# dusk-network/plonk

Measured on AMD Instinct MI355X. Metric: prove() wall-clock (ms) at 2^20 gates, lower is better.
Workload: dtype u32 limbs (Fr 256-bit / Fp 384-bit Montgomery)

## Files before the change

### plonk_amd/csrc/msm.hip

```cpp
#include <cstdlib>

#include "plonk_internal.hpp"
#include "curve28.cuh"
#include "fr29.cuh"

namespace plonk {


static constexpr uint32_t MSM_KSL = 32;
static constexpr uint32_t MSM_CHUNK = 16;

__device__ __forceinline__ Fr ld_fr_g(const Fr* p) {
  const uint4* q = reinterpret_cast<const uint4*>(p);
  uint4 a = q[0], b = q[1];
  Fr r;
  r.l[0] = a.x; r.l[1] = a.y; r.l[2] = a.z; r.l[3] = a.w;
  r.l[4] = b.x; r.l[5] = b.y; r.l[6] = b.z; r.l[7] = b.w;
  return r;
}
__device__ __forceinline__ Fp ld_fp(const Fp* p) {
  const uint4* q = reinterpret_cast<const uint4*>(p);
  uint4 a = q[0], b = q[1], c = q[2];
  Fp r;
  r.l[0] = a.x; r.l[1] = a.y; r.l[2] = a.z; r.l[3] = a.w;
// ... 410 lines not shown
  G1RSlot* __restrict__ buckets = buckets_all + (uint64_t)kb * MSM_NB;
  __shared__ G1R sh[BS_G > 1 ? 128 : 32];
  if (blockIdx.x < fused) {
    __shared__ uint32_t found[3];
    const HeavyItem* __restrict__ list = heavy_list_all + (uint64_t)kb * MSM_NB;
    G1RSlot* __restrict__ seg_sum = seg_sum_all + (uint64_t)kb * seg_cap;
    const uint32_t t = threadIdx.x, q = t & 3, L = t >> 2;
    const uint32_t nitems = nheavy_all[2 * kb], nsegs = nheavy_all[2 * kb + 1];
    for (uint32_t sg = blockIdx.x; sg < nsegs; sg += fused) {
      for (uint32_t i = t; i < nitems; i += 128) {
        const HeavyItem it = list[i];
        if (sg >= it.seg_base && sg < it.seg_base + it.nseg) { found[0] = it.bucket; found[1] = sg - it.seg_base; found[2] = it.nseg; }
      }
      __syncthreads();
      const uint32_t b = found[0], j = found[1], nseg = found[2];
      const uint32_t beg = slice_off[b] + j * HEAVY_SEG, bend = slice_off[b + 1];
      G1R acc = G1R::identity();
      for (uint32_t r = 0; r < HEAVY_SEG / 32; ++r) {
        const uint32_t k = beg + L + 32 * r;
        if (k < bend) acc = g1r_add_quad(acc, ld_g1r(partial + k), q);
      }
      for (uint32_t d = 16; d >= 1; d >>= 1) {
        if (q == 0) sh[L] = acc;
        __syncthreads();
        if (L < d) acc = g1r_add_quad(acc, sh[L + d], q);
        __syncthreads();
      }
      if (t == 0) st_g1r(nseg == 1 ? buckets + b : seg_sum + sg, acc);
      __syncthreads();
    }
    return;
  }
  if (multi_list_all || dense_quad) {
    const uint32_t nmulti = dense_quad ? MSM_NB : nheavy_all[2 * MSM_MAX_BATCH + kb];
    const uint32_t* __restrict__ list = multi_list_all ? multi_list_all + (uint64_t)kb * MSM_NB : nullptr;
    const uint32_t q = threadIdx.x & 3;
    for (uint32_t i = ((blockIdx.x - fused) * blockDim.x + threadIdx.x) >> 2; i < nmulti; i += ((gridDim.x - fused) * blockDim.x) >> 2) {
      const uint32_t mb = dense_quad ? i : list[i];
      const uint32_t beg = slice_off[mb], end = slice_off[mb + 1];
      if (dense_quad) {
        if (end - beg > heavy_thresh || (direct && end - beg == 1)) continue;
        if (end == beg) { if (q == 0) st_g1r(buckets + mb, G1R::identity()); continue; }
      }
      G1R acc = ld_g1r(partial + beg);
      for (uint32_t k = beg + 1; k < end; ++k) acc = g1r_add_quad(acc, ld_g1r(partial + k), q);
      if (q == 0) st_g1r(buckets + mb, acc);
    }
    return;
  }
  const uint32_t t = (blockIdx.x - fused) * blockDim.x + threadIdx.x;
  const uint32_t b = t / BS_G, g = t % BS_G;
  G1R acc = G1R::identity();
  bool heavy = false;
  if (b < MSM_NB) {
    const uint32_t beg = slice_off[b], end = slice_off[b + 1];
    heavy = end - beg > heavy_thresh;
    if (direct && end - beg == 1) heavy = true;
    if (!heavy)
      for (uint32_t k = beg + g; k < end; k += BS_G) acc = acc.add(ld_g1r(partial + k));
  }
  for (int d = BS_G / 2; d >= 1; d >>= 1) {
    sh[threadIdx.x] = acc;
    __syncthreads();
    if ((int)g < d) acc = acc.add(sh[threadIdx.x + d]);
    __syncthreads();
  }
  if (g == 0 && b < MSM_NB && !heavy) st_g1r(buckets + b, acc);
}

// ... 785 lines not shown
  }
  prof_end(c, 2);
  HIP_TRY(hipGetLastError());
  return PLONK_OK;
#endif
#undef FINE_BEGIN
#undef FINE_END
}


}

#if PLONK_MSM_NB_BITS == 15
static uint64_t msm_slice_cap(const Ctx* c, uint64_t cap) {
  if (c->cfg.ksl >= 4) return (uint64_t)MSM_W * cap / c->cfg.ksl + MSM_NB_MAX + 1;
  const uint64_t nb15 = 1ull << 15;
  const uint64_t small = (uint64_t)MSM_W * cap / 4 < (uint64_t)MSM_W * nb15 ? (uint64_t)MSM_W * cap / 4 : (uint64_t)MSM_W * nb15;
  const uint64_t large = (uint64_t)MSM_W * cap / MSM_KSL;
  return (small > large ? small : large) + MSM_NB_MAX + 1;
}

int msm_sort_reserve_fixed(Ctx* c) {
  MsmWork& w = c->msm;
  constexpr int KB = MSM_MAX_BATCH;
  constexpr uint32_t COARSE = 2048;
  HIP_TRY(hipMalloc((void**)&w.coarse_cnt, sizeof(uint32_t) * COARSE * KB));
  HIP_TRY(hipMalloc((void**)&w.coarse_off, sizeof(uint32_t) * (COARSE + 1) * KB));
  HIP_TRY(hipMalloc((void**)&w.coarse_cur, sizeof(uint32_t) * COARSE * KB));
  HIP_TRY(hipMalloc((void**)&w.big_off, sizeof(uint32_t) * (COARSE + 1) * KB));
  HIP_TRY(hipMalloc((void**)&w.big_cnt, sizeof(uint32_t) * 2 * MSM_NB_MAX * KB));
  HIP_TRY(hipMalloc((void**)&w.full_off, sizeof(uint32_t) * (MSM_NB_MAX + 1) * KB));
  HIP_TRY(hipMalloc((void**)&w.part_list, sizeof(uint32_t) * (MSM_NB_MAX + 1) * KB));
  HIP_TRY(hipMalloc((void**)&w.multi_list, sizeof(uint32_t) * MSM_NB_MAX * KB));
  HIP_TRY(hipMalloc((void**)&w.layout, sizeof(uint32_t) * (2 * (MSM_NB_MAX / 1024) + (MSM_NB_MAX / 1024 + 1) * 132) * KB));
  return PLONK_OK;
}

int msm_reserve(Ctx* c, uint64_t m) {
  MsmWork& w = c->msm;
  constexpr int KB = MSM_MAX_BATCH;
  if (!w.fixed_ok) {
    for (void** q : {(void**)&w.offsets, (void**)&w.slice_off, (void**)&w.nheavy, &w.heavy_list, (void**)&w.coarse_cnt, (void**)&w.coarse_off,
                     (void**)&w.coarse_cur, (void**)&w.big_off, (void**)&w.big_cnt, (void**)&w.full_off, (void**)&w.part_list, (void**)&w.layout, (void**)&w.multi_list, &w.buckets, &w.chunk,
                     (void**)&w.result}) {
      if (*q) { (void)hipFree(*q); *q = nullptr; }
    }
    if (w.result_host) { (void)hipHostFree(w.result_host); w.result_host = nullptr; }
    HIP_TRY(hipMalloc((void**)&w.offsets, sizeof(uint32_t) * (MSM_NB_MAX + 1) * KB));
    HIP_TRY(hipMalloc((void**)&w.slice_off, sizeof(uint32_t) * (MSM_NB_MAX + 1) * KB));
    HIP_TRY(hipMalloc((void**)&w.nheavy, sizeof(uint32_t) * 4 * KB));
    HIP_TRY(hipMalloc((void**)&w.heavy_list, sizeof(HeavyItem) * MSM_NB_MAX * KB));
    { const int rc_s = msm_sort_reserve_fixed(c); if (rc_s) return rc_s; }
    HIP_TRY(hipMalloc((void**)&w.buckets, sizeof(G1RSlot) * MSM_NB_MAX * KB));
    HIP_TRY(hipMalloc((void**)&w.chunk, sizeof(G1RSlot) * (2 * (MSM_NB_MAX / 128) + 1024) * KB));
    HIP_TRY(hipMalloc((void**)&w.result, sizeof(G1) * MSM_BIT_SUMS * KB));
    HIP_TRY(hipHostMalloc((void**)&w.result_host, sizeof(G1) * MSM_BIT_SUMS * KB, hipHostMallocDefault));
    w.fixed_ok = true;
  }
  if (m > w.cap_m || msm_slice_cap(c, w.cap_m) > w.cap_slices) {
    const uint64_t cap = m > w.cap_m ? m : w.cap_m;
    HIP_TRY(hipStreamSynchronize(c->stream));
    w.cap_m = 0;
    for (void** q : {(void**)&w.tmp_words, (void**)&w.entries, (void**)&w.partial, &w.seg_sum}) {
      if (*q) { HIP_TRY(hipFree(*q)); *q = nullptr; }
    }
    HIP_TRY(hipMalloc((void**)&w.tmp_words, sizeof(uint64_t) * MSM_W * cap * KB));
    HIP_TRY(hipMalloc((void**)&w.entries, sizeof(uint32_t) * MSM_W * cap * KB));
// ... 115 lines not shown
```

### plonk_amd/csrc/msm_sort.hip

```cpp
#include "plonk_internal.hpp"
#include "fr29.cuh"

namespace plonk {
namespace PLONK_MSM_NS {

static constexpr uint32_t FINE_BITS = MSM_NB_BITS - 11;
static constexpr uint32_t COARSE = MSM_NB >> FINE_BITS;
#ifndef PLONK_SORT_TILE
#define PLONK_SORT_TILE 2048
#endif
static constexpr uint32_t TILE = PLONK_SORT_TILE;
static constexpr uint32_t SORT_T = 1024;
static constexpr uint32_t PER_T = TILE / SORT_T;
#ifndef PLONK_HIST_PER
#define PLONK_HIST_PER 2
#endif
static constexpr uint32_t HIST_PER = PLONK_HIST_PER;
static constexpr uint32_t HIST_TILE = SORT_T * HIST_PER;
static_assert(COARSE == 2 * SORT_T, "scan / reservation loops assume two coarse bins per thread");
static constexpr uint32_t IDX_BITS = 31 - FINE_BITS;
static constexpr uint32_t IDX_MASK = (1u << IDX_BITS) - 1;
static_assert(IDX_BITS + 1 + FINE_BITS == 32, "narrow intermediate word layout");
template <class WordT> struct SortWord;
template <> struct SortWord<uint32_t> {
// ... 94 lines not shown
__device__ __forceinline__ uint32_t block_exclusive_scan(uint32_t v, uint32_t* sh , uint32_t* total) {
  const uint32_t t = threadIdx.x;
  sh[t] = v;
  __syncthreads();
  for (uint32_t d = 1; d < SORT_T; d <<= 1) {
    const uint32_t x = t >= d ? sh[t - d] : 0;
    __syncthreads();
    sh[t] += x;
    __syncthreads();
  }
  const uint32_t incl = sh[t];
  *total = sh[SORT_T - 1];
  __syncthreads();
  return incl - v;
}

__device__ __forceinline__ void fine_exclusive_scan(const uint32_t* cnt, uint32_t* ex, uint32_t* sc, uint32_t* total) {
  constexpr uint32_t NF = 1u << FINE_BITS;
  const uint32_t t = threadIdx.x;
  const uint32_t v = t < NF ? cnt[t] : 0u;
  if (t < NF) sc[t] = v;
  __syncthreads();
  for (uint32_t d = 1; d < NF; d <<= 1) {
    const uint32_t x = (t < NF && t >= d) ? sc[t - d] : 0u;
    __syncthreads();
    if (t < NF) sc[t] += x;
    __syncthreads();
  }
  if (t < NF) ex[t] = sc[t] - v;
  *total = sc[NF - 1];
  __syncthreads();
}

static constexpr uint32_t BIG_LIMIT = 1u << 16;
static constexpr uint32_t BIG_CHUNK = 1u << 14;
__device__ __forceinline__ uint32_t big_chunks(uint32_t cnt) { return cnt > BIG_LIMIT ? (cnt + BIG_CHUNK - 1) / BIG_CHUNK : 0u; }

__global__ void __launch_bounds__(SORT_T) msm_coarse_scan_kernel(const uint32_t* __restrict__ coarse_cnt_all,
                                                                 uint32_t* __restrict__ coarse_off_all,
                                                                 uint32_t* __restrict__ coarse_cur_all,
                                                                 uint32_t* __restrict__ big_off_all, int kb0) {
  __shared__ uint32_t sh[SORT_T];
  const uint32_t* __restrict__ cnt = coarse_cnt_all + (uint64_t)(blockIdx.x + (uint32_t)kb0) * COARSE;
  uint32_t* __restrict__ off = coarse_off_all + (uint64_t)(blockIdx.x + (uint32_t)kb0) * (COARSE + 1);
  uint32_t* __restrict__ cur = coarse_cur_all + (uint64_t)(blockIdx.x + (uint32_t)kb0) * COARSE;
  uint32_t* __restrict__ big = big_off_all + (uint64_t)(blockIdx.x + (uint32_t)kb0) * (COARSE + 1);
  const uint32_t t = threadIdx.x;
  const uint32_t c0 = cnt[2 * t], c1 = cnt[2 * t + 1];
  uint32_t total;
  const uint32_t ex = block_exclusive_scan(c0 + c1, sh, &total);
  off[2 * t] = ex;
  off[2 * t + 1] = ex + c0;
  cur[2 * t] = 0;
  cur[2 * t + 1] = 0;
  if (t == SORT_T - 1) off[COARSE] = total;
  const uint32_t b0 = big_chunks(c0), b1 = big_chunks(c1);
  uint32_t btotal;
  const uint32_t bex = block_exclusive_scan(b0 + b1, sh, &btotal);
  big[2 * t] = bex;
  big[2 * t + 1] = bex + b0;
  if (t == SORT_T - 1) big[COARSE] = btotal;
}

static constexpr size_t PARTITION_LDS = ((size_t)TILE * MSM_W + 3 * COARSE) * sizeof(uint32_t);

template <int MODE, class WordT>
// ... 157 lines not shown
    }
  }
  __syncthreads();
  const TmpPlanes<WordT> tmp(tmp_all, kb, (uint64_t)MSM_W * bt.cap_m);
#pragma unroll
  for (uint32_t k = 0; k < P2_PER; ++k)
#pragma unroll
    for (uint32_t w = 0; w < P2_W; ++w)
      if (where[k][w] != 0xffffffffu) stage[loff[where[k][w] >> 16] + (where[k][w] & 0xffffu)] = word[k][w];
  __syncthreads();
  const uint32_t sub = t & 7;
  for (uint32_t bin = t >> 3; bin < COARSE; bin += P2_T / 8) {
    const uint32_t cnt = hist[bin], lo = loff[bin], gb = gbase[bin];
    for (uint32_t j = sub; j < cnt; j += 8) {
      const uint32_t lw = stage[lo + j];
      tmp.st(gb + j, SortWord<WordT>::make(lw >> 20, (lw >> 19) & 1u, (uint64_t)((lw >> 11) & 0xffu) * srs_n + base + (lw & 0x7ffu)));
    }
  }
}
#endif

#ifndef PLONK_FINE_T
#define PLONK_FINE_T 512
#endif
#ifndef PLONK_FINE_CACHE
#define PLONK_FINE_CACHE 20
#endif
static constexpr uint32_t FINE_T = PLONK_FINE_T;
static constexpr uint32_t FINE_CACHE = PLONK_FINE_CACHE;
template <class WordT>
__global__ void __launch_bounds__(FINE_T) msm_fine_kernel(MsmBatch bt, const uint32_t* __restrict__ coarse_off_all,
                                                          void* __restrict__ tmp_all,
                                                          uint32_t* __restrict__ entries_all,
                                                          uint32_t* __restrict__ offsets_all) {
  __shared__ uint32_t cnt[1u << FINE_BITS], start[1u << FINE_BITS], cur[1u << FINE_BITS], scan_tmp[1u << FINE_BITS];
  const int kb = (int)blockIdx.y + bt.kb0;
  const uint32_t bin = blockIdx.x, t = threadIdx.x;
  const uint32_t* __restrict__ coff = coarse_off_all + (uint64_t)kb * (COARSE + 1);
  const TmpPlanes<WordT> tmp(tmp_all, kb, (uint64_t)MSM_W * bt.cap_m);
  uint32_t* __restrict__ entries = entries_all + (uint64_t)kb * MSM_W * bt.cap_m;
  uint32_t* __restrict__ offsets = offsets_all + (uint64_t)kb * (MSM_NB + 1);
  const uint32_t beg = coff[bin], end = coff[bin + 1];
  if (end - beg > BIG_LIMIT) return;
  if (t < (1u << FINE_BITS)) { cnt[t] = 0; cur[t] = 0; }
  __syncthreads();
  WordT cache[FINE_CACHE > 0 ? FINE_CACHE : 1];
#pragma unroll
  for (uint32_t r = 0; r < FINE_CACHE; ++r) {
    const uint32_t j = beg + t + r * FINE_T;
    cache[r] = j < end ? tmp.ld(j) : (WordT)0;
  }
#pragma unroll
  for (uint32_t r = 0; r < FINE_CACHE; ++r)
    if (beg + t + r * FINE_T < end) atomicAdd(&cnt[SortWord<WordT>::fine(cache[r])], 1u);
  for (uint32_t j = beg + t + FINE_CACHE * FINE_T; j < end; j += FINE_T) atomicAdd(&cnt[tmp.ld_fine(j)], 1u);
  __syncthreads();
  {
    uint32_t total;
    fine_exclusive_scan(cnt, start, scan_tmp, &total);
    if (t < (1u << FINE_BITS)) {
      start[t] += beg;
      offsets[(bin << FINE_BITS) + t] = start[t];
    }
    if (t == 0 && bin == COARSE - 1) offsets[MSM_NB] = beg + total;
    __syncthreads();
  }
  __shared__ uint32_t sorted[(MSM_NB_BITS > 15 && FINE_CACHE > 0) ? FINE_T * FINE_CACHE : 1];
  const bool staged = MSM_NB_BITS > 15 && FINE_CACHE > 0 && end - beg <= FINE_T * FINE_CACHE;
  auto place = [&](WordT e) {
    const uint32_t f = SortWord<WordT>::fine(e);
    const uint32_t pos = start[f] + atomicAdd(&cur[f], 1u);
    if (staged) sorted[pos - beg] = SortWord<WordT>::entry(e);
    else entries[pos] = SortWord<WordT>::entry(e);
  };
#pragma unroll
  for (uint32_t r = 0; r < FINE_CACHE; ++r)
    if (beg + t + r * FINE_T < end) place(cache[r]);
  for (uint32_t j = beg + t + FINE_CACHE * FINE_T; j < end; j += FINE_T) place(tmp.ld(j));
  if (staged) {
    __syncthreads();
    for (uint32_t j = t; j < end - beg; j += FINE_T) entries[beg + j] = sorted[j];
  }
}

__device__ __forceinline__ bool big_item(const uint32_t* __restrict__ big, const uint32_t* __restrict__ coff, uint32_t w,
                                         uint32_t* bin, uint32_t* beg, uint32_t* end) {
  if (w >= big[COARSE]) return false;
  uint32_t lo = 0, hi = COARSE - 1;
  while (lo < hi) {
    const uint32_t mid = (lo + hi + 1) >> 1;
    if (big[mid] <= w) lo = mid; else hi = mid - 1;
  }
// ... 1 lines not shown
  const uint32_t b0 = coff[lo] + (w - big[lo]) * BIG_CHUNK, b1 = coff[lo + 1];
  *beg = b0;
  *end = b0 + BIG_CHUNK < b1 ? b0 + BIG_CHUNK : b1;
  return true;
}
static constexpr uint32_t BIG_T = 512;
static constexpr uint32_t BIG_PER = BIG_CHUNK / BIG_T;
template <class WordT>
__global__ void __launch_bounds__(BIG_T) msm_big_hist_kernel(MsmBatch bt, const uint32_t* __restrict__ coarse_off_all,
                                                             const uint32_t* __restrict__ big_off_all,
                                                             void* __restrict__ tmp_all, uint32_t* __restrict__ big_cnt_all) {
  __shared__ uint32_t cnt[1u << FINE_BITS];
  const int kb = (int)blockIdx.y + bt.kb0;
  const uint32_t* __restrict__ coff = coarse_off_all + (uint64_t)kb * (COARSE + 1);
  const uint32_t* __restrict__ big = big_off_all + (uint64_t)kb * (COARSE + 1);
  const TmpPlanes<WordT> tmp(tmp_all, kb, (uint64_t)MSM_W * bt.cap_m);
  const uint32_t t = threadIdx.x;
  for (uint32_t item = blockIdx.x;; item += gridDim.x) {
    uint32_t bin, beg, end;
    if (!big_item(big, coff, item, &bin, &beg, &end)) return;
    if (t < (1u << FINE_BITS)) cnt[t] = 0;
    __syncthreads();
    for (uint32_t j = beg + t; j < end; j += BIG_T) atomicAdd(&cnt[tmp.ld_fine(j)], 1u);
    __syncthreads();
    if (t < (1u << FINE_BITS) && cnt[t]) atomicAdd(&big_cnt_all[(uint64_t)kb * MSM_NB + (bin << FINE_BITS) + t], cnt[t]);
    __syncthreads();
  }
}
template <class WordT>
__global__ void __launch_bounds__(BIG_T) msm_big_scatter_kernel(MsmBatch bt, const uint32_t* __restrict__ coarse_off_all,
                                                                const uint32_t* __restrict__ big_off_all,
                                                                void* __restrict__ tmp_all,
                                                                const uint32_t* __restrict__ big_cnt_all, uint32_t* __restrict__ big_cur_all,
                                                                uint32_t* __restrict__ entries_all, uint32_t* __restrict__ offsets_all) {
  __shared__ uint32_t cnt[1u << FINE_BITS], base[1u << FINE_BITS], cur[1u << FINE_BITS], bin_cnt[1u << FINE_BITS], scan_tmp[1u << FINE_BITS];
  const int kb = (int)blockIdx.y + bt.kb0;
  const uint32_t* __restrict__ coff = coarse_off_all + (uint64_t)kb * (COARSE + 1);
  const uint32_t* __restrict__ big = big_off_all + (uint64_t)kb * (COARSE + 1);
  const TmpPlanes<WordT> tmp(tmp_all, kb, (uint64_t)MSM_W * bt.cap_m);
  uint32_t* __restrict__ entries = entries_all + (uint64_t)kb * MSM_W * bt.cap_m;
  uint32_t* __restrict__ offsets = offsets_all + (uint64_t)kb * (MSM_NB + 1);
  const uint32_t t = threadIdx.x;
  for (uint32_t item = blockIdx.x;; item += gridDim.x) {
    uint32_t bin, beg, end;
    if (!big_item(big, coff, item, &bin, &beg, &end)) return;
    const uint32_t* __restrict__ bcnt = big_cnt_all + (uint64_t)kb * MSM_NB + (bin << FINE_BITS);
    uint32_t* __restrict__ bcur = big_cur_all + (uint64_t)kb * MSM_NB + (bin << FINE_BITS);
    if (t < (1u << FINE_BITS)) { cnt[t] = 0; cur[t] = 0; }
    __syncthreads();
    WordT cache[BIG_PER];
#pragma unroll
    for (uint32_t r = 0; r < BIG_PER; ++r) {
      const uint32_t j = beg + t + r * BIG_T;
      cache[r] = j < end ? tmp.ld(j) : (WordT)0;
      if (j < end) atomicAdd(&cnt[SortWord<WordT>::fine(cache[r])], 1u);
    }
    __syncthreads();
    {
      const bool first = beg == coff[bin];
      if (t < (1u << FINE_BITS)) bin_cnt[t] = bcnt[t];
      __syncthreads();
      uint32_t total;
      fine_exclusive_scan(bin_cnt, base, scan_tmp, &total);
      if (t < (1u << FINE_BITS)) {
        const uint32_t run = coff[bin] + base[t];
        if (first) offsets[(bin << FINE_BITS) + t] = run;
        base[t] = run + (cnt[t] ? atomicAdd(&bcur[t], cnt[t]) : 0u);
      }
      if (first && t == 0 && bin == COARSE - 1) offsets[MSM_NB] = coff[bin] + total;
    }
    __syncthreads();
#pragma unroll
    for (uint32_t r = 0; r < BIG_PER; ++r) {
      if (beg + t + r * BIG_T < end) {
        const WordT e = cache[r];
        const uint32_t f = SortWord<WordT>::fine(e);
        entries[base[f] + atomicAdd(&cur[f], 1u)] = SortWord<WordT>::entry(e);
      }
    }
    __syncthreads();
  }
}

static constexpr uint32_t HEAVY_SEG_SLICES = 128;
static constexpr uint32_t SLICES_STAGE_WORDS = MSM_NB + MSM_NB / 32 + 2;
static constexpr size_t SLICES_LDS = sizeof(uint32_t) * SLICES_STAGE_WORDS;
__device__ __forceinline__ uint32_t stage_at(uint32_t i) { return i + (i >> 5); }
template <bool ORDER>
__global__ void __launch_bounds__(SORT_T) msm_slices_kernel(const uint32_t* __restrict__ offsets_all,
                                                            uint32_t* __restrict__ slice_off_all, uint32_t ksl, uint32_t heavy_thresh,
                                                            uint32_t* __restrict__ nheavy_all, HeavyItem* __restrict__ heavy_list_all, int kb0,
                                                            uint32_t* __restrict__ full_off_all, uint32_t* __restrict__ part_list_all) {
  extern __shared__ __attribute__((aligned(16))) uint32_t stage[];
  __shared__ uint32_t sh[SORT_T];
  __shared__ uint32_t hist[129];
  const uint32_t* __restrict__ offsets = offsets_all + (uint64_t)(blockIdx.x + (uint32_t)kb0) * (MSM_NB + 1);
// ... 36 lines not shown
    uint32_t* __restrict__ part_list = part_list_all + (uint64_t)(blockIdx.x + (uint32_t)kb0) * (MSM_NB + 1);
    uint32_t mine_f = 0;
#pragma unroll
    for (uint32_t k = 0; k < PER; ++k) {
      const uint32_t c = o[k + 1] - o[k];
      mine_f += c >> sh_ksl;
      const uint32_t r = c & (ksl - 1);
      if (r) atomicAdd(&hist[r], 1u);
    }
    uint32_t total_f;
    uint32_t run_f = block_exclusive_scan(mine_f, sh, &total_f);
#pragma unroll
    for (uint32_t k = 0; k < PER; ++k) {
      stage[stage_at(t * PER + k)] = run_f;
      run_f += (o[k + 1] - o[k]) >> sh_ksl;
    }
    if (t == 0) {
      uint32_t acc = 0;
      for (uint32_t r = ksl - 1; r >= 1; --r) { const uint32_t h = hist[r]; hist[r] = acc; acc += h; }
      hist[0] = acc;
    }
    __syncthreads();
    for (uint32_t i = t; i < MSM_NB; i += SORT_T) full_off[i] = stage[stage_at(i)];
    if (t == SORT_T - 1) full_off[MSM_NB] = total_f;
#pragma unroll
    for (uint32_t k = 0; k < PER; ++k) {
      const uint32_t r = (o[k + 1] - o[k]) & (ksl - 1);
      if (r) part_list[atomicAdd(&hist[r], 1u)] = t * PER + k;
    }
    if (t == 0) part_list[MSM_NB] = hist[0];
  }
}
#if PLONK_MSM_NB_BITS > 15
static constexpr uint32_t LAY_NBLK = MSM_NB / SORT_T, LAY_H = 132;
static constexpr uint32_t LAY_WORDS = 2 * LAY_NBLK + (LAY_NBLK + 1) * LAY_H;
__global__ void __launch_bounds__(SORT_T) msm_layout_count_kernel(const uint32_t* __restrict__ offsets_all, uint32_t* __restrict__ slice_off_all,
                                                                  uint32_t* __restrict__ full_off_all, uint32_t* __restrict__ lay_all, uint32_t ksl, int kb0) {
  __shared__ uint32_t sh[SORT_T];
  __shared__ uint32_t hist[LAY_H];
  const int kb = (int)blockIdx.y + kb0;
  const uint32_t blk = blockIdx.x, t = threadIdx.x, b = blk * SORT_T + t;
  const uint32_t* __restrict__ offsets = offsets_all + (uint64_t)kb * (MSM_NB + 1);
  uint32_t* __restrict__ lay = lay_all + (uint64_t)kb * LAY_WORDS;
  if (t < LAY_H) hist[t] = 0;
  __syncthreads();
  const uint32_t cnt = offsets[b + 1] - offsets[b];
  const uint32_t nf = cnt / ksl, r = cnt % ksl, ns = nf + (r ? 1u : 0u);
  if (r) atomicAdd(&hist[r], 1u);
  uint32_t tot_ns, tot_nf;
  const uint32_t ex_ns = block_exclusive_scan(ns, sh, &tot_ns);
  const uint32_t ex_nf = block_exclusive_scan(nf, sh, &tot_nf);
  slice_off_all[(uint64_t)kb * (MSM_NB + 1) + b] = ex_ns;
  full_off_all[(uint64_t)kb * (MSM_NB + 1) + b] = ex_nf;
  if (t == 0) { lay[blk] = tot_ns; lay[LAY_NBLK + blk] = tot_nf; }
  if (t < LAY_H) lay[2 * LAY_NBLK + blk * LAY_H + t] = hist[t];
}
__global__ void __launch_bounds__(SORT_T) msm_layout_scan_kernel(uint32_t* __restrict__ slice_off_all, uint32_t* __restrict__ full_off_all,
                                                                 uint32_t* __restrict__ part_list_all, uint32_t* __restrict__ lay_all, uint32_t ksl, int kb0) {
  __shared__ uint32_t sh[SORT_T];
  __shared__ uint32_t ctot[LAY_H];
  const int kb = (blockIdx.x + (uint32_t)kb0);
  const uint32_t t = threadIdx.x;
  uint32_t* __restrict__ lay = lay_all + (uint64_t)kb * LAY_WORDS;
  static_assert(LAY_NBLK <= SORT_T, "one thread per block total");
  uint32_t tot;
  const uint32_t a = t < LAY_NBLK ? lay[t] : 0u;
  const uint32_t ea = block_exclusive_scan(a, sh, &tot);
  if (t < LAY_NBLK) lay[t] = ea;
  if (t == 0) slice_off_all[(uint64_t)kb * (MSM_NB + 1) + MSM_NB] = tot;
  const uint32_t f = t < LAY_NBLK ? lay[LAY_NBLK + t] : 0u;
  const uint32_t ef = block_exclusive_scan(f, sh, &tot);
  if (t < LAY_NBLK) lay[LAY_NBLK + t] = ef;
  if (t == 0) full_off_all[(uint64_t)kb * (MSM_NB + 1) + MSM_NB] = tot;
  if (t < LAY_H) {
    uint32_t run = 0;
    if (t >= 1 && t < ksl)
      for (uint32_t blk = 0; blk < LAY_NBLK; ++blk) {
        uint32_t* q = lay + 2 * LAY_NBLK + blk * LAY_H + t;
        const uint32_t h = *q;
        *q = run;
        run += h;
      }
    ctot[t] = run;
  }
  __syncthreads();
  if (t == 0) {
    uint32_t acc = 0;
    uint32_t* cstart = lay + 2 * LAY_NBLK + LAY_NBLK * LAY_H;
    for (uint32_t r = ksl - 1; r >= 1; --r) { cstart[r] = acc; acc += ctot[r]; }
    part_list_all[(uint64_t)kb * (MSM_NB + 1) + MSM_NB] = acc;
  }
}
__global__ void __launch_bounds__(SORT_T) msm_layout_apply_kernel(const uint32_t* __restrict__ offsets_all, uint32_t* __restrict__ slice_off_all,
                                                                  uint32_t* __restrict__ full_off_all, uint32_t* __restrict__ part_list_all,
                                                                  const uint32_t* __restrict__ lay_all, uint32_t ksl, uint32_t heavy_thresh,
                                                                  uint32_t* __restrict__ nheavy_all, HeavyItem* __restrict__ heavy_list_all,
                                                                  uint4* __restrict__ buckets_raw, uint32_t* __restrict__ multi_list_all, int kb0) {
  __shared__ uint32_t rank[LAY_H];
  const int kb = (int)blockIdx.y + kb0;
  const uint32_t blk = blockIdx.x, t = threadIdx.x, b = blk * SORT_T + t;
  const uint32_t* __restrict__ offsets = offsets_all + (uint64_t)kb * (MSM_NB + 1);
  const uint32_t* __restrict__ lay = lay_all + (uint64_t)kb * LAY_WORDS;
  if (t < LAY_H) rank[t] = 0;
  __syncthreads();
  const uint32_t cnt = offsets[b + 1] - offsets[b];
  const uint32_t nf = cnt / ksl, r = cnt % ksl, ns = nf + (r ? 1u : 0u);
  slice_off_all[(uint64_t)kb * (MSM_NB + 1) + b] += lay[blk];
  full_off_all[(uint64_t)kb * (MSM_NB + 1) + b] += lay[LAY_NBLK + blk];
  if (r) {
    const uint32_t pos = lay[2 * LAY_NBLK + LAY_NBLK * LAY_H + r] + lay[2 * LAY_NBLK + blk * LAY_H + r] + atomicAdd(&rank[r], 1u);
    part_list_all[(uint64_t)kb * (MSM_NB + 1) + pos] = b;
  }
  if (ns > heavy_thresh) {
    HeavyItem it;
    it.bucket = b;
    it.nseg = (ns + HEAVY_SEG_SLICES - 1) / HEAVY_SEG_SLICES;
    it.seg_base = atomicAdd(&nheavy_all[2 * kb + 1], it.nseg);
    it.pad = 0;
    heavy_list_all[(uint64_t)kb * MSM_NB + atomicAdd(&nheavy_all[2 * kb], 1u)] = it;
  } else if (ns == 0) {
    uint4* q = buckets_raw + ((uint64_t)kb * MSM_NB + b) * 16;
#pragma unroll
    for (int k = 0; k < 16; ++k) q[k] = make_uint4(0u, 0u, 0u, 0u);
  }
  __shared__ uint32_t nmul, mbase;
  if (t == 0) nmul = 0;
  __syncthreads();
  const bool multi = ns >= 2 && ns <= heavy_thresh;
  const uint32_t mrank = multi ? atomicAdd(&nmul, 1u) : 0u;
  __syncthreads();
  if (t == 0 && nmul) mbase = atomicAdd(&nheavy_all[2 * MSM_MAX_BATCH + kb], nmul);
  __syncthreads();
  if (multi) multi_list_all[(uint64_t)kb * MSM_NB + mbase + mrank] = b;
}
#endif

int msm_order_slices(Ctx* c, const MsmBatch& bt) {
  (void)c; (void)bt;
  return PLONK_OK;
}

template <int MODE, class WordT>
static int msm_group_sort_t(Ctx* c, const MsmBatch& bt, uint64_t mmax) {
  MsmWork& w = c->msm;
  hipStream_t st = c->stream;
  const uint32_t tiles = (uint32_t)((mmax + TILE - 1) / TILE);
  const uint32_t htiles = (uint32_t)((mmax + HIST_TILE - 1) / HIST_TILE);
  void* tmp = (void*)w.tmp_words;
  const int kb0 = bt.kb0;
  HIP_TRY(hipMemsetAsync(w.coarse_cnt + (size_t)COARSE * kb0, 0, sizeof(uint32_t) * COARSE * bt.count, st));
  hipLaunchKernelGGL(msm_hist_kernel<MODE>, dim3(htiles, bt.count), dim3(SORT_T), 0, st, bt, w.coarse_cnt);
  hipLaunchKernelGGL(msm_coarse_scan_kernel, dim3(bt.count), dim3(SORT_T), 0, st, w.coarse_cnt, w.coarse_off, w.coarse_cur, w.big_off, kb0);
#if PLONK_MSM_NB_BITS >= 19
  if constexpr (MODE == 1 || MODE == 2) {
    if (c->cfg.sort13 == 1) {
      const uint32_t tiles2 = (uint32_t)((mmax + P2_TILE - 1) / P2_TILE);
      smem_opt_in(c, (const void*)msm_partition2_kernel<MODE, WordT>, PARTITION2_LDS);
      hipLaunchKernelGGL((msm_partition2_kernel<MODE, WordT>), dim3(tiles2, bt.count), dim3(P2_T), PARTITION2_LDS, st, bt, bt.table_n,
                         w.coarse_off, w.coarse_cur, tmp);
    }
  }
  if (MODE == 0 || MODE == 3 || c->cfg.sort13 != 1) {
#else
  {
#endif
    smem_opt_in(c, (const void*)msm_partition_kernel<MODE, WordT>, PARTITION_LDS);
    hipLaunchKernelGGL((msm_partition_kernel<MODE, WordT>), dim3(tiles, bt.count), dim3(SORT_T), PARTITION_LDS, st, bt, bt.table_n,
                       w.coarse_off, w.coarse_cur, tmp);
  }
  hipLaunchKernelGGL(msm_fine_kernel<WordT>, dim3(COARSE, bt.count), dim3(FINE_T), 0, st, bt, w.coarse_off, tmp,
                     w.entries, w.offsets);
  {
    const uint64_t words = (uint64_t)MSM_W * mmax;
    const uint32_t most = (uint32_t)(words / BIG_CHUNK + words / BIG_LIMIT + 1);
    const uint32_t big_wgs = most < 512u ? most : 512u;
    if (kb0 == 0 && bt.count == bt.group_count) {
      HIP_TRY(hipMemsetAsync(w.big_cnt, 0, sizeof(uint32_t) * 2 * MSM_NB * MSM_MAX_BATCH, st));
    } else {
      HIP_TRY(hipMemsetAsync(w.big_cnt + (size_t)MSM_NB * kb0, 0, sizeof(uint32_t) * MSM_NB * bt.count, st));
      HIP_TRY(hipMemsetAsync(w.big_cnt + (size_t)MSM_NB * MSM_MAX_BATCH + (size_t)MSM_NB * kb0, 0, sizeof(uint32_t) * MSM_NB * bt.count, st));
    }
    hipLaunchKernelGGL(msm_big_hist_kernel<WordT>, dim3(big_wgs, bt.count), dim3(BIG_T), 0, st, bt, w.coarse_off, w.big_off, tmp, w.big_cnt);
    hipLaunchKernelGGL(msm_big_scatter_kernel<WordT>, dim3(big_wgs, bt.count), dim3(BIG_T), 0, st, bt, w.coarse_off, w.big_off, tmp,
                       w.big_cnt, w.big_cnt + (size_t)MSM_NB * MSM_MAX_BATCH, w.entries, w.offsets);
  }
  if (kb0 == 0 && bt.count == bt.group_count) {
    HIP_TRY(hipMemsetAsync(w.nheavy, 0, sizeof(uint32_t) * 4 * MSM_MAX_BATCH, st));
  } else {
    HIP_TRY(hipMemsetAsync(w.nheavy + 2 * kb0, 0, sizeof(uint32_t) * 2 * bt.count, st));
    HIP_TRY(hipMemsetAsync(w.nheavy + 2 * MSM_MAX_BATCH + kb0, 0, sizeof(uint32_t) * bt.count, st));
  }
#if PLONK_MSM_NB_BITS > 15
  if (bt.ksl > 128) return (set_last_error("msm_group_sort", "slice length above 128", __FILE__, __LINE__), PLONK_ERR_ARG);
  hipLaunchKernelGGL(msm_layout_count_kernel, dim3(LAY_NBLK, bt.count), dim3(SORT_T), 0, st, w.offsets, w.slice_off, w.full_off, w.layout, bt.ksl, kb0);
  hipLaunchKernelGGL(msm_layout_scan_kernel, dim3(bt.count), dim3(SORT_T), 0, st, w.slice_off, w.full_off, w.part_list, w.layout, bt.ksl, kb0);
  hipLaunchKernelGGL(msm_layout_apply_kernel, dim3(LAY_NBLK, bt.count), dim3(SORT_T), 0, st, w.offsets, w.slice_off, w.full_off, w.part_list,
                     (const uint32_t*)w.layout, bt.ksl, bt.heavy_thresh, w.nheavy, (HeavyItem*)w.heavy_list, (uint4*)w.buckets, w.multi_list, kb0);
#else
  if (bt.ordered) {
    if (bt.ksl > 128) return (set_last_error("msm_group_sort", "slice length above 128", __FILE__, __LINE__), PLONK_ERR_ARG);
    smem_opt_in(c, (const void*)msm_slices_kernel<true>, SLICES_LDS);
    hipLaunchKernelGGL(msm_slices_kernel<true>, dim3(bt.count), dim3(SORT_T), SLICES_LDS, st, w.offsets, w.slice_off, bt.ksl, bt.heavy_thresh,
                       w.nheavy, (HeavyItem*)w.heavy_list, kb0, w.full_off, w.part_list);
  } else {
    smem_opt_in(c, (const void*)msm_slices_kernel<false>, SLICES_LDS);
    hipLaunchKernelGGL(msm_slices_kernel<false>, dim3(bt.count), dim3(SORT_T), SLICES_LDS, st, w.offsets, w.slice_off, bt.ksl, bt.heavy_thresh,
                       w.nheavy, (HeavyItem*)w.heavy_list, kb0, (uint32_t*)nullptr, (uint32_t*)nullptr);
  }
#endif
  HIP_TRY(hipGetLastError());
  return PLONK_OK;
}
int msm_group_sort(Ctx* c, const MsmBatch& bt, uint64_t mmax) {
  if ((uint64_t)bt.rows * bt.table_n > (1ull << 31))
    return (set_last_error("commit key too large for the bucket sort", "table rows * points must be <= 2^31", __FILE__, __LINE__), PLONK_ERR_ARG);
  if (bt.rows == MSM_ROWS_BITPOS) return bt.wide ? msm_group_sort_t<1, uint64_t>(c, bt, mmax) : msm_group_sort_t<1, uint32_t>(c, bt, mmax);
  if (bt.rows == MSM_ROWS_HALFPOS) return bt.wide ? msm_group_sort_t<2, uint64_t>(c, bt, mmax) : msm_group_sort_t<2, uint32_t>(c, bt, mmax);
  if (bt.rows == MSM_ROWS_QUARTERPOS) return bt.wide ? msm_group_sort_t<3, uint64_t>(c, bt, mmax) : msm_group_sort_t<3, uint32_t>(c, bt, mmax);
#if PLONK_MSM_NB_BITS == 15
  return bt.wide ? msm_group_sort_t<0, uint64_t>(c, bt, mmax) : msm_group_sort_t<0, uint32_t>(c, bt, mmax);
#else
  return (set_last_error("msm_group_sort", "window tables need the 2^15-bucket variant", __FILE__, __LINE__), PLONK_ERR_ARG);
#endif
}
bool msm_needs_wide_words(uint32_t rows, uint64_t table_n) { return (uint64_t)rows * table_n > (1ull << IDX_BITS); }

}
}
```

Before: 30.74.

## Fuse MSM slice layout counting into fine sort and tree-reduce long multi buckets

Computes the per-bucket slice and full-slice scans and the remainder histogram inside the fine and big-scatter sort kernels, which removes the separate layout count kernel and its re-read of offsets. The layout scan is parallelised across eight partitions per remainder column instead of one serial walk per column. Multi-slice buckets are split into two lists: buckets with more than two slices are reduced by eight cooperating quads with a shared-memory tree, while two-slice buckets keep the one-quad-per-bucket path. This adds LDS scans and barriers to the sort kernels and requires the slice length to be a power of two.

After: 30.69, median of 4. About the same (-0.2%).

```diff
diff --git a/plonk_amd/csrc/msm.hip b/plonk_amd/csrc/msm.hip
--- a/plonk_amd/csrc/msm.hip
+++ b/plonk_amd/csrc/msm.hip
@@ -466,9 +466,33 @@
     return;
   }
   if (multi_list_all || dense_quad) {
-    const uint32_t nmulti = dense_quad ? MSM_NB : nheavy_all[2 * MSM_MAX_BATCH + kb];
+    const uint32_t nmulti = dense_quad ? MSM_NB : nheavy_all[2 * MSM_MAX_BATCH + 2 * kb];
     const uint32_t* __restrict__ list = multi_list_all ? multi_list_all + (uint64_t)kb * MSM_NB : nullptr;
     const uint32_t q = threadIdx.x & 3;
+#if PLONK_MSM_NB_BITS > 15
+    if (!dense_quad) {
+      const uint32_t ntree = nheavy_all[2 * MSM_MAX_BATCH + 2 * kb + 1];
+      const uint32_t nwg = gridDim.x - fused, wg = blockIdx.x - fused;
+      const uint32_t quad = threadIdx.x >> 2, j = quad & 7;
+      for (uint32_t i0 = 0; i0 < ntree; i0 += 4 * nwg) {
+        const uint32_t i = i0 + (quad >> 3) * nwg + wg;
+        G1R acc = G1R::identity();
+        uint32_t mb = 0;
+        if (i < ntree) {
+          mb = list[MSM_NB - 1 - i];
+          const uint32_t beg = slice_off[mb], end = slice_off[mb + 1];
+          for (uint32_t k = beg + j; k < end; k += 8) acc = g1r_add_quad(acc, ld_g1r(partial + k), q);
+        }
+        for (uint32_t d = 4; d >= 1; d >>= 1) {
+          if (q == 0) sh[quad] = acc;
+          __syncthreads();
+          if (j < d) acc = g1r_add_quad(acc, sh[quad + d], q);
+          __syncthreads();
+        }
+        if (i < ntree && j == 0 && q == 0) st_g1r(buckets + mb, acc);
+      }
+    }
+#endif
     for (uint32_t i = ((blockIdx.x - fused) * blockDim.x + threadIdx.x) >> 2; i < nmulti; i += ((gridDim.x - fused) * blockDim.x) >> 2) {
       const uint32_t mb = dense_quad ? i : list[i];
       const uint32_t beg = slice_off[mb], end = slice_off[mb + 1];
@@ -1320,7 +1344,7 @@
   HIP_TRY(hipMalloc((void**)&w.full_off, sizeof(uint32_t) * (MSM_NB_MAX + 1) * KB));
   HIP_TRY(hipMalloc((void**)&w.part_list, sizeof(uint32_t) * (MSM_NB_MAX + 1) * KB));
   HIP_TRY(hipMalloc((void**)&w.multi_list, sizeof(uint32_t) * MSM_NB_MAX * KB));
-  HIP_TRY(hipMalloc((void**)&w.layout, sizeof(uint32_t) * (2 * (MSM_NB_MAX / 1024) + (MSM_NB_MAX / 1024 + 1) * 132) * KB));
+  HIP_TRY(hipMalloc((void**)&w.layout, sizeof(uint32_t) * (2 * 2048 + (2048 + 1) * 132) * KB));
   return PLONK_OK;
 }
 
diff --git a/plonk_amd/csrc/msm_sort.hip b/plonk_amd/csrc/msm_sort.hip
--- a/plonk_amd/csrc/msm_sort.hip
+++ b/plonk_amd/csrc/msm_sort.hip
@@ -150,6 +150,53 @@
   __syncthreads();
 }
 
+#if PLONK_MSM_NB_BITS > 15
+static constexpr uint32_t LAY_NBLK = COARSE, LAY_BLK = 1u << FINE_BITS, LAY_H = 132;
+static constexpr uint32_t LAY_WORDS = 2 * LAY_NBLK + (LAY_NBLK + 1) * LAY_H;
+struct LayoutOut {
+  uint32_t* slice_off;
+  uint32_t* full_off;
+  uint32_t* lay;
+};
+__device__ __forceinline__ LayoutOut layout_out(uint32_t* slice_off_all, uint32_t* full_off_all, uint32_t* lay_all, int kb) {
+  return LayoutOut{slice_off_all + (uint64_t)kb * (MSM_NB + 1), full_off_all + (uint64_t)kb * (MSM_NB + 1), lay_all + (uint64_t)kb * LAY_WORDS};
+}
+__device__ __forceinline__ void fine_layout_scan(const uint32_t* cnt, uint32_t ksl, uint32_t* ex, uint32_t* sc, uint32_t* sc_ns, uint32_t* sc_nf,
+                                                 uint32_t* hist , uint32_t* total) {
+  constexpr uint32_t NF = 1u << FINE_BITS;
+  const uint32_t t = threadIdx.x;
+  const uint32_t sh_ksl = 31u - (uint32_t)__builtin_clz(ksl);
+  const uint32_t v = t < NF ? cnt[t] : 0u;
+  const uint32_t nf = v >> sh_ksl, r = v & (ksl - 1u), ns = nf + (r ? 1u : 0u);
+  if (t < NF) { sc[t] = v; sc_ns[t] = ns; sc_nf[t] = nf; }
+  if (t < LAY_H) hist[t] = 0;
+  __syncthreads();
+  if (t < NF && r) atomicAdd(&hist[r], 1u);
+  for (uint32_t d = 1; d < NF; d <<= 1) {
+    const bool on = t < NF && t >= d;
+    const uint32_t x = on ? sc[t - d] : 0u, xs = on ? sc_ns[t - d] : 0u, xf = on ? sc_nf[t - d] : 0u;
+    __syncthreads();
+    if (t < NF) { sc[t] += x; sc_ns[t] += xs; sc_nf[t] += xf; }
+    __syncthreads();
+  }
+  if (t < NF) ex[t] = sc[t] - v;
+  *total = sc[NF - 1];
+  __syncthreads();
+}
+__device__ __forceinline__ void layout_block_store(const LayoutOut& lo, uint32_t bin, const uint32_t* cnt, uint32_t ksl, const uint32_t* sc_ns,
+                                                   const uint32_t* sc_nf, const uint32_t* hist) {
+  constexpr uint32_t NF = 1u << FINE_BITS;
+  const uint32_t t = threadIdx.x;
+  if (t < NF) {
+    const uint32_t v = cnt[t], nf = v / ksl, ns = nf + ((v & (ksl - 1u)) ? 1u : 0u);
+    lo.slice_off[(bin << FINE_BITS) + t] = sc_ns[t] - ns;
+    lo.full_off[(bin << FINE_BITS) + t] = sc_nf[t] - nf;
+  }
+  if (t == 0) { lo.lay[bin] = sc_ns[NF - 1]; lo.lay[LAY_NBLK + bin] = sc_nf[NF - 1]; }
+  if (t < LAY_H) lo.lay[2 * LAY_NBLK + bin * LAY_H + t] = hist[t];
+}
+#endif
+
 static constexpr uint32_t BIG_LIMIT = 1u << 16;
 static constexpr uint32_t BIG_CHUNK = 1u << 14;
 __device__ __forceinline__ uint32_t big_chunks(uint32_t cnt) { return cnt > BIG_LIMIT ? (cnt + BIG_CHUNK - 1) / BIG_CHUNK : 0u; }
@@ -373,8 +420,14 @@
 __global__ void __launch_bounds__(FINE_T) msm_fine_kernel(MsmBatch bt, const uint32_t* __restrict__ coarse_off_all,
                                                           void* __restrict__ tmp_all,
                                                           uint32_t* __restrict__ entries_all,
-                                                          uint32_t* __restrict__ offsets_all) {
+                                                          uint32_t* __restrict__ offsets_all,
+                                                          uint32_t* __restrict__ slice_off_all, uint32_t* __restrict__ full_off_all,
+                                                          uint32_t* __restrict__ lay_all ) {
   __shared__ uint32_t cnt[1u << FINE_BITS], start[1u << FINE_BITS], cur[1u << FINE_BITS], scan_tmp[1u << FINE_BITS];
+#if PLONK_MSM_NB_BITS > 15
+  static_assert(FINE_T >= (1u << FINE_BITS) && FINE_T >= LAY_H, "one thread per fine bucket and per remainder class");
+  __shared__ uint32_t scan_ns[1u << FINE_BITS], scan_nf[1u << FINE_BITS], lay_hist[LAY_H];
+#endif
   const int kb = (int)blockIdx.y + bt.kb0;
   const uint32_t bin = blockIdx.x, t = threadIdx.x;
   const uint32_t* __restrict__ coff = coarse_off_all + (uint64_t)kb * (COARSE + 1);
@@ -398,7 +451,12 @@
   __syncthreads();
   {
     uint32_t total;
+#if PLONK_MSM_NB_BITS > 15
+    fine_layout_scan(cnt, bt.ksl, start, scan_tmp, scan_ns, scan_nf, lay_hist, &total);
+    layout_block_store(layout_out(slice_off_all, full_off_all, lay_all, kb), bin, cnt, bt.ksl, scan_ns, scan_nf, lay_hist);
+#else
     fine_exclusive_scan(cnt, start, scan_tmp, &total);
+#endif
     if (t < (1u << FINE_BITS)) {
       start[t] += beg;
       offsets[(bin << FINE_BITS) + t] = start[t];
@@ -466,8 +524,14 @@
                                                                 const uint32_t* __restrict__ big_off_all,
                                                                 void* __restrict__ tmp_all,
                                                                 const uint32_t* __restrict__ big_cnt_all, uint32_t* __restrict__ big_cur_all,
-                                                                uint32_t* __restrict__ entries_all, uint32_t* __restrict__ offsets_all) {
+                                                                uint32_t* __restrict__ entries_all, uint32_t* __restrict__ offsets_all,
+                                                                uint32_t* __restrict__ slice_off_all, uint32_t* __restrict__ full_off_all,
+                                                                uint32_t* __restrict__ lay_all ) {
   __shared__ uint32_t cnt[1u << FINE_BITS], base[1u << FINE_BITS], cur[1u << FINE_BITS], bin_cnt[1u << FINE_BITS], scan_tmp[1u << FINE_BITS];
+#if PLONK_MSM_NB_BITS > 15
+  static_assert(BIG_T >= (1u << FINE_BITS) && BIG_T >= LAY_H, "one thread per fine bucket and per remainder class");
+  __shared__ uint32_t scan_ns[1u << FINE_BITS], scan_nf[1u << FINE_BITS], lay_hist[LAY_H];
+#endif
   const int kb = (int)blockIdx.y + bt.kb0;
   const uint32_t* __restrict__ coff = coarse_off_all + (uint64_t)kb * (COARSE + 1);
   const uint32_t* __restrict__ big = big_off_all + (uint64_t)kb * (COARSE + 1);
@@ -495,7 +559,12 @@
       if (t < (1u << FINE_BITS)) bin_cnt[t] = bcnt[t];
       __syncthreads();
       uint32_t total;
+#if PLONK_MSM_NB_BITS > 15
+      fine_layout_scan(bin_cnt, bt.ksl, base, scan_tmp, scan_ns, scan_nf, lay_hist, &total);
+      if (first) layout_block_store(layout_out(slice_off_all, full_off_all, lay_all, kb), bin, bin_cnt, bt.ksl, scan_ns, scan_nf, lay_hist);
+#else
       fine_exclusive_scan(bin_cnt, base, scan_tmp, &total);
+#endif
       if (t < (1u << FINE_BITS)) {
         const uint32_t run = coff[bin] + base[t];
         if (first) offsets[(bin << FINE_BITS) + t] = run;
@@ -598,62 +667,48 @@
   }
 }
 #if PLONK_MSM_NB_BITS > 15
-static constexpr uint32_t LAY_NBLK = MSM_NB / SORT_T, LAY_H = 132;
-static constexpr uint32_t LAY_WORDS = 2 * LAY_NBLK + (LAY_NBLK + 1) * LAY_H;
-__global__ void __launch_bounds__(SORT_T) msm_layout_count_kernel(const uint32_t* __restrict__ offsets_all, uint32_t* __restrict__ slice_off_all,
-                                                                  uint32_t* __restrict__ full_off_all, uint32_t* __restrict__ lay_all, uint32_t ksl, int kb0) {
-  __shared__ uint32_t sh[SORT_T];
-  __shared__ uint32_t hist[LAY_H];
-  const int kb = (int)blockIdx.y + kb0;
-  const uint32_t blk = blockIdx.x, t = threadIdx.x, b = blk * SORT_T + t;
-  const uint32_t* __restrict__ offsets = offsets_all + (uint64_t)kb * (MSM_NB + 1);
-  uint32_t* __restrict__ lay = lay_all + (uint64_t)kb * LAY_WORDS;
-  if (t < LAY_H) hist[t] = 0;
-  __syncthreads();
-  const uint32_t cnt = offsets[b + 1] - offsets[b];
-  const uint32_t nf = cnt / ksl, r = cnt % ksl, ns = nf + (r ? 1u : 0u);
-  if (r) atomicAdd(&hist[r], 1u);
-  uint32_t tot_ns, tot_nf;
-  const uint32_t ex_ns = block_exclusive_scan(ns, sh, &tot_ns);
-  const uint32_t ex_nf = block_exclusive_scan(nf, sh, &tot_nf);
-  slice_off_all[(uint64_t)kb * (MSM_NB + 1) + b] = ex_ns;
-  full_off_all[(uint64_t)kb * (MSM_NB + 1) + b] = ex_nf;
-  if (t == 0) { lay[blk] = tot_ns; lay[LAY_NBLK + blk] = tot_nf; }
-  if (t < LAY_H) lay[2 * LAY_NBLK + blk * LAY_H + t] = hist[t];
-}
+static_assert(LAY_NBLK == 2 * SORT_T, "two block totals per thread");
+static constexpr uint32_t LAY_PARTS = SORT_T / 128, LAY_PART_BLKS = LAY_NBLK / LAY_PARTS;
 __global__ void __launch_bounds__(SORT_T) msm_layout_scan_kernel(uint32_t* __restrict__ slice_off_all, uint32_t* __restrict__ full_off_all,
                                                                  uint32_t* __restrict__ part_list_all, uint32_t* __restrict__ lay_all, uint32_t ksl, int kb0) {
   __shared__ uint32_t sh[SORT_T];
-  __shared__ uint32_t ctot[LAY_H];
+  __shared__ uint32_t ctot[128];
   const int kb = (blockIdx.x + (uint32_t)kb0);
   const uint32_t t = threadIdx.x;
   uint32_t* __restrict__ lay = lay_all + (uint64_t)kb * LAY_WORDS;
-  static_assert(LAY_NBLK <= SORT_T, "one thread per block total");
   uint32_t tot;
-  const uint32_t a = t < LAY_NBLK ? lay[t] : 0u;
-  const uint32_t ea = block_exclusive_scan(a, sh, &tot);
-  if (t < LAY_NBLK) lay[t] = ea;
+  const uint32_t a0 = lay[2 * t], a1 = lay[2 * t + 1];
+  const uint32_t ea = block_exclusive_scan(a0 + a1, sh, &tot);
+  lay[2 * t] = ea;
+  lay[2 * t + 1] = ea + a0;
   if (t == 0) slice_off_all[(uint64_t)kb * (MSM_NB + 1) + MSM_NB] = tot;
-  const uint32_t f = t < LAY_NBLK ? lay[LAY_NBLK + t] : 0u;
-  const uint32_t ef = block_exclusive_scan(f, sh, &tot);
-  if (t < LAY_NBLK) lay[LAY_NBLK + t] = ef;
+  const uint32_t f0 = lay[LAY_NBLK + 2 * t], f1 = lay[LAY_NBLK + 2 * t + 1];
+  const uint32_t ef = block_exclusive_scan(f0 + f1, sh, &tot);
+  lay[LAY_NBLK + 2 * t] = ef;
+  lay[LAY_NBLK + 2 * t + 1] = ef + f0;
   if (t == 0) full_off_all[(uint64_t)kb * (MSM_NB + 1) + MSM_NB] = tot;
-  if (t < LAY_H) {
-    uint32_t run = 0;
-    if (t >= 1 && t < ksl)
-      for (uint32_t blk = 0; blk < LAY_NBLK; ++blk) {
-        uint32_t* q = lay + 2 * LAY_NBLK + blk * LAY_H + t;
-        const uint32_t h = *q;
-        *q = run;
-        run += h;
-      }
-    ctot[t] = run;
-  }
+  const uint32_t part = t >> 7, r = t & 127u;
+  const bool live = r >= 1 && r < ksl;
+  uint32_t* const col = lay + 2 * LAY_NBLK + (uint64_t)part * LAY_PART_BLKS * LAY_H + r;
+  uint32_t sum = 0;
+  if (live)
+    for (uint32_t blk = 0; blk < LAY_PART_BLKS; ++blk) sum += col[blk * LAY_H];
+  sh[t] = sum;
+  __syncthreads();
+  uint32_t run = 0;
+  for (uint32_t p = 0; p < part; ++p) run += sh[p * 128 + r];
+  if (part == LAY_PARTS - 1) ctot[r] = run + sum;
+  if (live)
+    for (uint32_t blk = 0; blk < LAY_PART_BLKS; ++blk) {
+      const uint32_t h = col[blk * LAY_H];
+      col[blk * LAY_H] = run;
+      run += h;
+    }
   __syncthreads();
   if (t == 0) {
     uint32_t acc = 0;
     uint32_t* cstart = lay + 2 * LAY_NBLK + LAY_NBLK * LAY_H;
-    for (uint32_t r = ksl - 1; r >= 1; --r) { cstart[r] = acc; acc += ctot[r]; }
+    for (uint32_t c = ksl - 1; c >= 1; --c) { cstart[c] = acc; acc += ctot[c]; }
     part_list_all[(uint64_t)kb * (MSM_NB + 1) + MSM_NB] = acc;
   }
 }
@@ -662,19 +717,20 @@
                                                                   const uint32_t* __restrict__ lay_all, uint32_t ksl, uint32_t heavy_thresh,
                                                                   uint32_t* __restrict__ nheavy_all, HeavyItem* __restrict__ heavy_list_all,
                                                                   uint4* __restrict__ buckets_raw, uint32_t* __restrict__ multi_list_all, int kb0) {
-  __shared__ uint32_t rank[LAY_H];
+  constexpr uint32_t SUBS = SORT_T / LAY_BLK;
+  __shared__ uint32_t rank[SUBS * LAY_H];
   const int kb = (int)blockIdx.y + kb0;
-  const uint32_t blk = blockIdx.x, t = threadIdx.x, b = blk * SORT_T + t;
+  const uint32_t t = threadIdx.x, b = blockIdx.x * SORT_T + t, blk = b >> FINE_BITS, sub = t >> FINE_BITS;
   const uint32_t* __restrict__ offsets = offsets_all + (uint64_t)kb * (MSM_NB + 1);
   const uint32_t* __restrict__ lay = lay_all + (uint64_t)kb * LAY_WORDS;
-  if (t < LAY_H) rank[t] = 0;
+  for (uint32_t i = t; i < SUBS * LAY_H; i += SORT_T) rank[i] = 0;
   __syncthreads();
   const uint32_t cnt = offsets[b + 1] - offsets[b];
   const uint32_t nf = cnt / ksl, r = cnt % ksl, ns = nf + (r ? 1u : 0u);
   slice_off_all[(uint64_t)kb * (MSM_NB + 1) + b] += lay[blk];
   full_off_all[(uint64_t)kb * (MSM_NB + 1) + b] += lay[LAY_NBLK + blk];
   if (r) {
-    const uint32_t pos = lay[2 * LAY_NBLK + LAY_NBLK * LAY_H + r] + lay[2 * LAY_NBLK + blk * LAY_H + r] + atomicAdd(&rank[r], 1u);
+    const uint32_t pos = lay[2 * LAY_NBLK + LAY_NBLK * LAY_H + r] + lay[2 * LAY_NBLK + blk * LAY_H + r] + atomicAdd(&rank[sub * LAY_H + r], 1u);
     part_list_all[(uint64_t)kb * (MSM_NB + 1) + pos] = b;
   }
   if (ns > heavy_thresh) {
@@ -689,15 +745,19 @@
 #pragma unroll
     for (int k = 0; k < 16; ++k) q[k] = make_uint4(0u, 0u, 0u, 0u);
   }
-  __shared__ uint32_t nmul, mbase;
-  if (t == 0) nmul = 0;
+  __shared__ uint32_t nmul[2], mbase[2];
+  if (t < 2) nmul[t] = 0;
   __syncthreads();
   const bool multi = ns >= 2 && ns <= heavy_thresh;
-  const uint32_t mrank = multi ? atomicAdd(&nmul, 1u) : 0u;
-  __syncthreads();
-  if (t == 0 && nmul) mbase = atomicAdd(&nheavy_all[2 * MSM_MAX_BATCH + kb], nmul);
-  __syncthreads();
-  if (multi) multi_list_all[(uint64_t)kb * MSM_NB + mbase + mrank] = b;
+  const uint32_t which = ns > 2 ? 1u : 0u;
+  const uint32_t mrank = multi ? atomicAdd(&nmul[which], 1u) : 0u;
+  __syncthreads();
+  if (t < 2 && nmul[t]) mbase[t] = atomicAdd(&nheavy_all[2 * MSM_MAX_BATCH + 2 * kb + t], nmul[t]);
+  __syncthreads();
+  if (multi) {
+    const uint32_t at = mbase[which] + mrank;
+    multi_list_all[(uint64_t)kb * MSM_NB + (which ? MSM_NB - 1 - at : at)] = b;
+  }
 }
 #endif
 
@@ -714,6 +774,9 @@
   const uint32_t htiles = (uint32_t)((mmax + HIST_TILE - 1) / HIST_TILE);
   void* tmp = (void*)w.tmp_words;
   const int kb0 = bt.kb0;
+#if PLONK_MSM_NB_BITS > 15
+  if (bt.ksl == 0 || bt.ksl > 128 || (bt.ksl & (bt.ksl - 1)) != 0) return (set_last_error("msm_group_sort", "slice length above 128 or no power of two", __FILE__, __LINE__), PLONK_ERR_ARG);
+#endif
   HIP_TRY(hipMemsetAsync(w.coarse_cnt + (size_t)COARSE * kb0, 0, sizeof(uint32_t) * COARSE * bt.count, st));
   hipLaunchKernelGGL(msm_hist_kernel<MODE>, dim3(htiles, bt.count), dim3(SORT_T), 0, st, bt, w.coarse_cnt);
   hipLaunchKernelGGL(msm_coarse_scan_kernel, dim3(bt.count), dim3(SORT_T), 0, st, w.coarse_cnt, w.coarse_off, w.coarse_cur, w.big_off, kb0);
@@ -735,7 +798,7 @@
                        w.coarse_off, w.coarse_cur, tmp);
   }
   hipLaunchKernelGGL(msm_fine_kernel<WordT>, dim3(COARSE, bt.count), dim3(FINE_T), 0, st, bt, w.coarse_off, tmp,
-                     w.entries, w.offsets);
+                     w.entries, w.offsets, w.slice_off, w.full_off, w.layout);
   {
     const uint64_t words = (uint64_t)MSM_W * mmax;
     const uint32_t most = (uint32_t)(words / BIG_CHUNK + words / BIG_LIMIT + 1);
@@ -748,19 +811,17 @@
     }
     hipLaunchKernelGGL(msm_big_hist_kernel<WordT>, dim3(big_wgs, bt.count), dim3(BIG_T), 0, st, bt, w.coarse_off, w.big_off, tmp, w.big_cnt);
     hipLaunchKernelGGL(msm_big_scatter_kernel<WordT>, dim3(big_wgs, bt.count), dim3(BIG_T), 0, st, bt, w.coarse_off, w.big_off, tmp,
-                       w.big_cnt, w.big_cnt + (size_t)MSM_NB * MSM_MAX_BATCH, w.entries, w.offsets);
+                       w.big_cnt, w.big_cnt + (size_t)MSM_NB * MSM_MAX_BATCH, w.entries, w.offsets, w.slice_off, w.full_off, w.layout);
   }
   if (kb0 == 0 && bt.count == bt.group_count) {
     HIP_TRY(hipMemsetAsync(w.nheavy, 0, sizeof(uint32_t) * 4 * MSM_MAX_BATCH, st));
   } else {
     HIP_TRY(hipMemsetAsync(w.nheavy + 2 * kb0, 0, sizeof(uint32_t) * 2 * bt.count, st));
-    HIP_TRY(hipMemsetAsync(w.nheavy + 2 * MSM_MAX_BATCH + kb0, 0, sizeof(uint32_t) * bt.count, st));
+    HIP_TRY(hipMemsetAsync(w.nheavy + 2 * MSM_MAX_BATCH + 2 * kb0, 0, sizeof(uint32_t) * 2 * bt.count, st));
   }
 #if PLONK_MSM_NB_BITS > 15
-  if (bt.ksl > 128) return (set_last_error("msm_group_sort", "slice length above 128", __FILE__, __LINE__), PLONK_ERR_ARG);
-  hipLaunchKernelGGL(msm_layout_count_kernel, dim3(LAY_NBLK, bt.count), dim3(SORT_T), 0, st, w.offsets, w.slice_off, w.full_off, w.layout, bt.ksl, kb0);
   hipLaunchKernelGGL(msm_layout_scan_kernel, dim3(bt.count), dim3(SORT_T), 0, st, w.slice_off, w.full_off, w.part_list, w.layout, bt.ksl, kb0);
-  hipLaunchKernelGGL(msm_layout_apply_kernel, dim3(LAY_NBLK, bt.count), dim3(SORT_T), 0, st, w.offsets, w.slice_off, w.full_off, w.part_list,
+  hipLaunchKernelGGL(msm_layout_apply_kernel, dim3(MSM_NB / SORT_T, bt.count), dim3(SORT_T), 0, st, w.offsets, w.slice_off, w.full_off, w.part_list,
                      (const uint32_t*)w.layout, bt.ksl, bt.heavy_thresh, w.nheavy, (HeavyItem*)w.heavy_list, (uint4*)w.buckets, w.multi_list, kb0);
 #else
   if (bt.ordered) {
```
